# lucidrains/imagen-pytorch

Hardware: AMD Instinct MI355X
Metric: images/sec (64->256 cascade, 1000 steps, bs=8) (higher is better)
Workload: dtype f16; 1 GPU; C3: README unet1 (dim 32, 64^2) + unet2 (dim 32, 256^2, lowres_cond) cascade, 1000 DDPM steps/stage, CFG 3.0, dynamic thresholding, batch 8 per GPU; global_batch=8, parallelism=batch-sharded x1, one RCCL all-gather of final images, batch_schedule=5 whole cascades side by side (one stream each), images_in_flight=40, denoiser_evals_per_image=4000

## Files before the change

imagen-pytorch_amd/csrc/attention.hip:

```cpp
#include <cstdlib>
#include <type_traits>
#include <utility>
#include "common.h"

namespace {

constexpr int KT = 32;
constexpr int KSTR = 144;
constexpr int VSTR = 72;

template <int D>
__global__ __launch_bounds__(256) void attention_kernel(const ImagenAttentionParams p) {
  constexpr int KS = D / 16;
  constexpr int DB = D / 32;
  constexpr int KSTRD = 2 * D + 16;
  constexpr int KBYTES = KT * KSTRD;
  constexpr int VBYTES = D * VSTR;
  __shared__ __attribute__((aligned(16))) char smem[2 * (KBYTES + VBYTES)];
  const int tid = threadIdx.x, lane = tid & 63, wave = tid >> 6;
  const int half = lane >> 5, l31 = lane & 31;
  const int b = blockIdx.z, hd = blockIdx.y;
  const int row = blockIdx.x * 128 + wave * 32 + l31;
  const int row_c = row < p.rows ? row : p.rows - 1;

  const f16* q = reinterpret_cast<const f16*>(p.q) + (size_t)b * p.q_bs + (size_t)hd * p.q_hs + (size_t)row_c * p.q_rs;
  f16x8 qf[KS];
#pragma unroll
  for (int s = 0; s < KS; ++s) qf[s] = *reinterpret_cast<const f16x8*>(q + 16 * s + 8 * half);
  if (p.q_scale) {
    float ssq = 0.f;
#pragma unroll
    for (int s = 0; s < KS; ++s)
#pragma unroll
      for (int j = 0; j < 8; ++j) ssq += (float)qf[s][j] * (float)qf[s][j];
    ssq += __shfl_xor(ssq, 32);
    const float inv = p.q_mult / fmaxf(sqrtf(ssq), 1e-12f);
#pragma unroll
    for (int s = 0; s < KS; ++s) {
      const float4 g0 = *reinterpret_cast<const float4*>(p.q_scale + 16 * s + 8 * half);
      const float4 g1 = *reinterpret_cast<const float4*>(p.q_scale + 16 * s + 8 * half + 4);
      const float g[8] = {g0.x, g0.y, g0.z, g0.w, g1.x, g1.y, g1.z, g1.w};
#pragma unroll
      for (int j = 0; j < 8; ++j) qf[s][j] = (f16)((float)qf[s][j] * inv * g[j]);
    }
  }

  const f16* kg = reinterpret_cast<const f16*>(p.k) + (size_t)b * p.k_bs + (size_t)hd * p.k_hs;
  const f16* vg = reinterpret_cast<const f16*>(p.vt) + (size_t)b * p.vt_bs + (size_t)hd * p.vt_hs;
  const bool stager = tid < 4 * D;
  const int sk_key = tid / (D / 8), sk_dg = tid % (D / 8);
  const int sv_d = (tid >> 2) & (D - 1), sv_kg = tid & 3;

  uint4 k_stage = make_uint4(0, 0, 0, 0), v_stage = make_uint4(0, 0, 0, 0);
  auto tile_load = [&](int kt0) {
    if (stager) {
      k_stage = *reinterpret_cast<const uint4*>(kg + (size_t)(kt0 + sk_key) * p.k_rs + sk_dg * 8);
      v_stage = *reinterpret_cast<const uint4*>(vg + (size_t)sv_d * p.vt_ds + kt0 + sv_kg * 8);
    }
  };
  auto tile_store = [&](char* buf) {
    if (stager) {
      *reinterpret_cast<uint4*>(buf + sk_key * KSTRD + sk_dg * 16) = k_stage;
      uint2* vd = reinterpret_cast<uint2*>(buf + KBYTES + sv_d * VSTR + sv_kg * 16);
      vd[0] = make_uint2(v_stage.x, v_stage.y);
      vd[1] = make_uint2(v_stage.z, v_stage.w);
    }
  };

  f32x16 oacc[DB];
#pragma unroll
  for (int db = 0; db < DB; ++db)
#pragma unroll
    for (int r = 0; r < 16; ++r) oacc[db][r] = 0.f;
  float m_run = -1.0e30f, l_run = 0.f;

  const int ntiles = (p.J + KT - 1) / KT;
  tile_load(0);
  tile_store(smem);
  __syncthreads();
  int cur = 0;
  for (int t = 0; t < ntiles; ++t) {
    const bool more = t + 1 < ntiles;
    if (more) tile_load((t + 1) * KT);
    const char* kb = smem + cur * (KBYTES + VBYTES);
    const char* vb = kb + KBYTES;

    f32x16 sacc;
#pragma unroll
    for (int r = 0; r < 16; ++r) sacc[r] = 0.f;
#pragma unroll
    for (int s = 0; s < KS; ++s) {
      const f16x8 kf = *reinterpret_cast<const f16x8*>(kb + l31 * KSTRD + (16 * s + 8 * half) * 2);
      sacc = __builtin_amdgcn_mfma_f32_32x32x16_f16(kf, qf[s], sacc, 0, 0, 0);
    }
    const int kbase = t * KT + 4 * half;
    float mx = -1.0e30f;
#pragma unroll
    for (int r = 0; r < 16; ++r) {
      const int key = kbase + (r & 3) + 8 * (r >> 2);
      if (key >= p.J) sacc[r] = -1.0e30f;
      mx = fmaxf(mx, sacc[r]);
    }
    mx = fmaxf(mx, __shfl_xor(mx, 32));
    const float m_new = fmaxf(m_run, mx);
    const float alpha = exp2f(m_run - m_new);
    m_run = m_new;
    float psum = 0.f;
    f16x8 pf[2], pl[2];
#pragma unroll
    for (int r = 0; r < 16; ++r) {
      const float e = exp2f(sacc[r] - m_new);
      psum += e;
      const f16 eh = (f16)e;
      pf[r >> 3][r & 7] = eh;
      pl[r >> 3][r & 7] = (f16)(e - (float)eh);
    }
    l_run = l_run * alpha + psum;
#pragma unroll
    for (int db = 0; db < DB; ++db)
#pragma unroll
      for (int r = 0; r < 16; ++r) oacc[db][r] *= alpha;

#pragma unroll
    for (int s = 0; s < 2; ++s) {
#pragma unroll
      for (int db = 0; db < DB; ++db) {
        const char* vrow = vb + (32 * db + l31) * VSTR + (16 * s + 4 * half) * 2;
        const uint2 lo = *reinterpret_cast<const uint2*>(vrow);
        const uint2 hi = *reinterpret_cast<const uint2*>(vrow + 16);
        uint4 packed = make_uint4(lo.x, lo.y, hi.x, hi.y);
        const f16x8 vf = *reinterpret_cast<const f16x8*>(&packed);
        oacc[db] = __builtin_amdgcn_mfma_f32_32x32x16_f16(vf, pl[s], oacc[db], 0, 0, 0);
        oacc[db] = __builtin_amdgcn_mfma_f32_32x32x16_f16(vf, pf[s], oacc[db], 0, 0, 0);
      }
    }

    if (more) tile_store(smem + (cur ^ 1) * (KBYTES + VBYTES));
    __syncthreads();
    cur ^= 1;
  }

  const float l_tot = l_run + __shfl_xor(l_run, 32);
  const float inv = 1.0f / l_tot;
  if (row < p.rows) {
    f16* o = reinterpret_cast<f16*>(p.o) + (size_t)b * p.o_bs + (size_t)hd * p.o_hs + (size_t)row * p.o_rs;
#pragma unroll
    for (int db = 0; db < DB; ++db)
#pragma unroll
      for (int qd = 0; qd < 4; ++qd) {
        f16x4 v;
#pragma unroll
        for (int e = 0; e < 4; ++e) v[e] = (f16)(oacc[db][4 * qd + e] * inv);
        *reinterpret_cast<f16x4*>(o + 32 * db + 8 * qd + 4 * half) = v;
      }
  }
}

constexpr int KT2 = 64;
constexpr int VSTR2 = 144;
constexpr int KBYTES2 = KT2 * KSTR;
constexpr int VBYTES2 = 64 * VSTR2;

template <int MINW, int SUB>
__global__ __launch_bounds__(512, MINW) void attention_kernel_w8(const ImagenAttentionParams p) {
  extern __shared__ __attribute__((aligned(16))) char smem[];
  constexpr int SLOT = KBYTES2 + VBYTES2;
  const int tid = threadIdx.x, lane = tid & 63, wave = tid >> 6;
  const int half = lane >> 5, l31 = lane & 31;
  const int b = blockIdx.z, hd = blockIdx.y;
  const int row = blockIdx.x * 256 + wave * 32 + l31;
  const int row_c = row < p.rows ? row : p.rows - 1;

  const f16* q = reinterpret_cast<const f16*>(p.q) + (size_t)b * p.q_bs + (size_t)hd * p.q_hs + (size_t)row_c * p.q_rs;
  f16x8 qf[4];
#pragma unroll
  for (int s = 0; s < 4; ++s) qf[s] = *reinterpret_cast<const f16x8*>(q + 16 * s + 8 * half);
  if (p.q_scale) {
    float ssq = 0.f;
#pragma unroll
    for (int s = 0; s < 4; ++s)
#pragma unroll
      for (int j = 0; j < 8; ++j) ssq += (float)qf[s][j] * (float)qf[s][j];
    ssq += __shfl_xor(ssq, 32);
    const float inv = p.q_mult / fmaxf(sqrtf(ssq), 1e-12f);
#pragma unroll
    for (int s = 0; s < 4; ++s) {
      const float4 g0 = *reinterpret_cast<const float4*>(p.q_scale + 16 * s + 8 * half);
      const float4 g1 = *reinterpret_cast<const float4*>(p.q_scale + 16 * s + 8 * half + 4);
      const float g[8] = {g0.x, g0.y, g0.z, g0.w, g1.x, g1.y, g1.z, g1.w};
#pragma unroll
      for (int j = 0; j < 8; ++j) qf[s][j] = (f16)((float)qf[s][j] * inv * g[j]);
    }
  }

  const f16* kg = reinterpret_cast<const f16*>(p.k) + (size_t)b * p.k_bs + (size_t)hd * p.k_hs;
  const f16* vg = reinterpret_cast<const f16*>(p.vt) + (size_t)b * p.vt_bs + (size_t)hd * p.vt_hs;
  const int sk_key = tid >> 3, sk_dg = tid & 7;
  const int sv_d = tid >> 3, sv_kg = tid & 7;
  const int Jpad = (p.J + 31) & ~31;
  const int ntiles = (p.J + KT2 - 1) / KT2;

  uint4 ks0, vs0, ks1, vs1;
  auto one_load = [&](int t, uint4& ks, uint4& vs) __attribute__((always_inline)) {
    const int kt0 = t < ntiles ? t * KT2 : 0;
    const int kk = kt0 + sk_key < Jpad ? kt0 + sk_key : kt0;
    const int kv = kt0 + sv_kg * 8 < Jpad ? kt0 + sv_kg * 8 : kt0;
    ks = *reinterpret_cast<const uint4*>(kg + (size_t)kk * p.k_rs + sk_dg * 8);
    vs = *reinterpret_cast<const uint4*>(vg + (size_t)sv_d * p.vt_ds + kv);
  };
  auto one_store = [&](char* buf, const uint4& ks, const uint4& vs) __attribute__((always_inline)) {
    *reinterpret_cast<uint4*>(buf + sk_key * KSTR + sk_dg * 16) = ks;
    char* vrow = buf + KBYTES2 + sv_d * VSTR2 + (sv_kg >> 1) * 32 + (sv_kg & 1) * 8;
    *reinterpret_cast<uint2*>(vrow) = make_uint2(vs.x, vs.y);
    *reinterpret_cast<uint2*>(vrow + 16) = make_uint2(vs.z, vs.w);
  };
  auto group_load = [&](int t0) __attribute__((always_inline)) {
    one_load(t0, ks0, vs0);
    if constexpr (SUB > 1) one_load(t0 + 1, ks1, vs1);
  };
  auto group_store = [&](char* buf) __attribute__((always_inline)) {
    one_store(buf, ks0, vs0);
    if constexpr (SUB > 1) one_store(buf + SLOT, ks1, vs1);
  };

  f32x16 oacc[2];
#pragma unroll
  for (int db = 0; db < 2; ++db)
#pragma unroll
    for (int r = 0; r < 16; ++r) oacc[db][r] = 0.f;
  float m_run = -1.0e30f, l_run = 0.f;

  group_load(0);
  group_store(smem);
  __syncthreads();
  int cur = 0;
  for (int t0 = 0; t0 < ntiles; t0 += SUB) {
    const bool more = t0 + SUB < ntiles;
    if (more) group_load(t0 + SUB);
#pragma unroll
    for (int u = 0; u < SUB; ++u) {
      const int t = t0 + u;
      if (u > 0 && t >= ntiles) continue;
      const char* kb = smem + (cur * SUB + u) * SLOT;
      const char* vb = kb + KBYTES2;

      f32x16 sacc[2];
#pragma unroll
      for (int h2 = 0; h2 < 2; ++h2) {
#pragma unroll
        for (int r = 0; r < 16; ++r) sacc[h2][r] = 0.f;
#pragma unroll
        for (int s = 0; s < 4; ++s) {
          const f16x8 kf = *reinterpret_cast<const f16x8*>(kb + (32 * h2 + l31) * KSTR + (16 * s + 8 * half) * 2);
          sacc[h2] = __builtin_amdgcn_mfma_f32_32x32x16_f16(kf, qf[s], sacc[h2], 0, 0, 0);
        }
      }
      if (t == ntiles - 1) {
#pragma unroll
        for (int h2 = 0; h2 < 2; ++h2)
#pragma unroll
          for (int r = 0; r < 16; ++r) {
            const int key = t * KT2 + 32 * h2 + 4 * half + (r & 3) + 8 * (r >> 2);
            if (key >= p.J) sacc[h2][r] = -1.0e30f;
          }
      }
      float mx = sacc[0][0];
#pragma unroll
      for (int h2 = 0; h2 < 2; ++h2)
#pragma unroll
        for (int r = 0; r < 16; ++r) mx = fmaxf(mx, sacc[h2][r]);
      mx = fmaxf(mx, __shfl_xor(mx, 32));
      const float m_new = fmaxf(m_run, mx);
      if (__any(m_new > m_run)) {
        const float alpha = __builtin_amdgcn_exp2f(m_run - m_new);
        l_run *= alpha;
#pragma unroll
        for (int db = 0; db < 2; ++db)
#pragma unroll
          for (int r = 0; r < 16; ++r) oacc[db][r] *= alpha;
        m_run = m_new;
      }
      float psum = 0.f;
      f16x8 pf[4];
#pragma unroll
      for (int h2 = 0; h2 < 2; ++h2)
#pragma unroll
        for (int r = 0; r < 16; ++r) {
          const float e = __builtin_amdgcn_exp2f(sacc[h2][r] - m_run);
          psum += e;
          pf[2 * h2 + (r >> 3)][r & 7] = (f16)e;
        }
      l_run += psum;

#pragma unroll
      for (int h2 = 0; h2 < 2; ++h2)
#pragma unroll
        for (int s = 0; s < 2; ++s) {
#pragma unroll
          for (int db = 0; db < 2; ++db) {
            const f16x8 vf = *reinterpret_cast<const f16x8*>(vb + (32 * db + l31) * VSTR2 + (32 * h2 + 16 * s + 8 * half) * 2);
            oacc[db] = __builtin_amdgcn_mfma_f32_32x32x16_f16(vf, pf[2 * h2 + s], oacc[db], 0, 0, 0);
          }
        }
    }
    if (more) group_store(smem + (cur ^ 1) * SUB * SLOT);
    __syncthreads();
    cur ^= 1;
  }

  const float l_tot = l_run + __shfl_xor(l_run, 32);
  const float inv = 1.0f / l_tot;
  if (row < p.rows) {
    f16* o = reinterpret_cast<f16*>(p.o) + (size_t)b * p.o_bs + (size_t)hd * p.o_hs + (size_t)row * p.o_rs;
#pragma unroll
    for (int db = 0; db < 2; ++db)
#pragma unroll
      for (int qd = 0; qd < 4; ++qd) {
        f16x4 v;
#pragma unroll
        for (int e = 0; e < 4; ++e) v[e] = (f16)(oacc[db][4 * qd + e] * inv);
        *reinterpret_cast<f16x4*>(o + 32 * db + 8 * qd + 4 * half) = v;
      }
  }
}

constexpr int BND_RING = 4;

template <class F, int... I>
__device__ __forceinline__ void att_static_for_impl(F&& f, std::integer_sequence<int, I...>) {
  (f(std::integral_constant<int, I>{}), ...);
}
template <int N, class F>
__device__ __forceinline__ void att_static_for(F&& f) {
  att_static_for_impl(static_cast<F&&>(f), std::make_integer_sequence<int, N>{});
}

struct AttFrag { f16x8 k[4], v[4]; };

__device__ __forceinline__ void att_frag_load(AttFrag& f, const char* krow, const char* vrow) {
#pragma unroll
  for (int s = 0; s < 4; ++s) f.k[s] = *reinterpret_cast<const f16x8*>(krow + 32 * s);
#pragma unroll
  for (int k = 0; k < 4; ++k) f.v[k] = *reinterpret_cast<const f16x8*>(vrow + (k & 1) * 32 * VSTR2 + (k >> 1) * 32);
}

template <bool QK, bool PV>
__device__ __forceinline__ void att_bnd_step(f32x16& Sn, f32x16& Sc, f16x8 (&pc)[2], const f16x8 (&pp)[2], f32x16 (&oacc)[2], float& sum0, float& sum1,
                                             const f16x8 (&qf)[4], const AttFrag& fc, AttFrag& fn, const char* krow_next, const char* vrow_next) {
  __builtin_amdgcn_sched_barrier(0);
  IMAGEN_OPAQUE(Sc);
  att_frag_load(fn, krow_next, vrow_next);
#pragma unroll
  for (int r = 0; r < 16; ++r) {
    const float e = __builtin_amdgcn_exp2f(Sc[r]);
    if (r & 1) sum1 += e; else sum0 += e;
    pc[r >> 3][r & 7] = (f16)e;
  }
  f32x16 zero;
#pragma unroll
  for (int r = 0; r < 16; ++r) zero[r] = 0.f;
#pragma unroll
  for (int k = 0; k < 4; ++k) {
    if constexpr (QK) Sn = __builtin_amdgcn_mfma_f32_32x32x16_f16(fc.k[k], qf[k], k == 0 ? zero : Sn, 0, 0, 0);
    if constexpr (PV) oacc[k & 1] = __builtin_amdgcn_mfma_f32_32x32x16_f16(fc.v[k], pp[k >> 1], oacc[k & 1], 0, 0, 0);
  }
  constexpr int NM = (QK ? 4 : 0) + (PV ? 4 : 0);
  att_static_for<NM>([&](auto kc) __attribute__((always_inline)) {
    __builtin_amdgcn_sched_group_barrier(0x008, 1, 0);
    __builtin_amdgcn_sched_group_barrier(0x100, 8 / NM, 0);
    __builtin_amdgcn_sched_group_barrier(0x400, 16 / NM, 0);
    __builtin_amdgcn_sched_group_barrier(0x002, NM == 8 ? 3 : 6, 0);
  });
  __builtin_amdgcn_sched_barrier(0);
}

template <int NW>
__global__ __launch_bounds__(64 * NW, 2) void attention_kernel_bnd(const ImagenAttentionParams p) {
  extern __shared__ __attribute__((aligned(16))) char smem[];
  constexpr int SLOT = KBYTES2 + VBYTES2;
  constexpr int NT = 64 * NW, IT = 512 / NT;
  static_assert(IT * NT == 512 && IT <= 2, "512 items per tile, one or two per thread");
  const int tid = threadIdx.x, lane = tid & 63, wave = tid >> 6;
  const int half = lane >> 5, l31 = lane & 31;
  const int b = blockIdx.z, hd = blockIdx.y;
  const int row = blockIdx.x * (32 * NW) + wave * 32 + l31;
  const int row_c = row < p.rows ? row : p.rows - 1;

  const f16* q = reinterpret_cast<const f16*>(p.q) + (size_t)b * p.q_bs + (size_t)hd * p.q_hs + (size_t)row_c * p.q_rs;
  f16x8 qf[4];
#pragma unroll
  for (int s = 0; s < 4; ++s) qf[s] = *reinterpret_cast<const f16x8*>(q + 16 * s + 8 * half);
  if (p.q_scale) {
    float ssq = 0.f;
#pragma unroll
    for (int s = 0; s < 4; ++s)
#pragma unroll
      for (int j = 0; j < 8; ++j) ssq += (float)qf[s][j] * (float)qf[s][j];
    ssq += __shfl_xor(ssq, 32);
    const float inv = p.q_mult / fmaxf(sqrtf(ssq), 1e-12f);
#pragma unroll
    for (int s = 0; s < 4; ++s) {
      const float4 g0 = *reinterpret_cast<const float4*>(p.q_scale + 16 * s + 8 * half);
      const float4 g1 = *reinterpret_cast<const float4*>(p.q_scale + 16 * s + 8 * half + 4);
      const float g[8] = {g0.x, g0.y, g0.z, g0.w, g1.x, g1.y, g1.z, g1.w};
#pragma unroll
      for (int j = 0; j < 8; ++j) qf[s][j] = (f16)((float)qf[s][j] * inv * g[j]);
    }
  }

  const f16* kg = reinterpret_cast<const f16*>(p.k) + (size_t)b * p.k_bs + (size_t)hd * p.k_hs;
  const f16* vg = reinterpret_cast<const f16*>(p.vt) + (size_t)b * p.vt_bs + (size_t)hd * p.vt_hs;
  const int Jpad = (p.J + 31) & ~31;
  const int ntiles = (p.J + KT2 - 1) / KT2;
  struct Stage { uint4 k0, v0, k1, v1; };
  Stage st0, st1;
  auto load_item = [&](int kt0, int i, uint4& kd, uint4& vd) __attribute__((always_inline)) {
    const int key = i >> 3, g8 = i & 7;
    const int kk = kt0 + key < Jpad ? kt0 + key : kt0;
    const int kv = kt0 + g8 * 8 < Jpad ? kt0 + g8 * 8 : kt0;
    kd = *reinterpret_cast<const uint4*>(kg + (size_t)kk * p.k_rs + g8 * 8);
    vd = *reinterpret_cast<const uint4*>(vg + (size_t)key * p.vt_ds + kv);
  };
  auto store_item = [&](char* buf, int i, const uint4& kd, const uint4& vd) __attribute__((always_inline)) {
    const int key = i >> 3, g8 = i & 7;
    *reinterpret_cast<uint4*>(buf + key * KSTR + g8 * 16) = kd;
    char* vrow = buf + KBYTES2 + key * VSTR2 + (g8 >> 1) * 32 + (g8 & 1) * 8;
    *reinterpret_cast<uint2*>(vrow) = make_uint2(vd.x, vd.y);
    *reinterpret_cast<uint2*>(vrow + 16) = make_uint2(vd.z, vd.w);
  };
  auto one_load = [&](int t, Stage& st) __attribute__((always_inline)) {
    const int kt0 = (t < ntiles ? t : ntiles - 1) * KT2;
    load_item(kt0, tid, st.k0, st.v0);
    if constexpr (IT > 1) load_item(kt0, tid + NT, st.k1, st.v1);
  };
  auto one_store = [&](char* buf, const Stage& st) __attribute__((always_inline)) {
    store_item(buf, tid, st.k0, st.v0);
    if constexpr (IT > 1) store_item(buf, tid + NT, st.k1, st.v1);
  };
  auto slot = [&](int t) __attribute__((always_inline)) { return smem + (t & (BND_RING - 1)) * SLOT; };
  const int koff = l31 * KSTR + 16 * half, voff = KBYTES2 + l31 * VSTR2 + 16 * half;
  auto krow = [&](int t, int hh) __attribute__((always_inline)) { return slot(t) + koff + hh * 32 * KSTR; };
  auto vrow = [&](int t, int hh) __attribute__((always_inline)) { return slot(t) + voff + hh * 64; };
  auto mask_last = [&](f32x16& S, int t, int hh) __attribute__((always_inline)) {
#pragma unroll
    for (int r = 0; r < 16; ++r) {
      const int key = t * KT2 + 32 * hh + 4 * half + (r & 3) + 8 * (r >> 2);
      if (key >= p.J) S[r] = -1.0e30f;
    }
  };

  f32x16 oacc[2], S0, S1;
#pragma unroll
  for (int db = 0; db < 2; ++db)
#pragma unroll
    for (int r = 0; r < 16; ++r) oacc[db][r] = 0.f;
  f16x8 pA[2], pB[2];
#pragma unroll
  for (int s = 0; s < 2; ++s)
#pragma unroll
    for (int j = 0; j < 8; ++j) pA[s][j] = pB[s][j] = (f16)0.f;
  float sum0 = 0.f, sum1 = 0.f;
  AttFrag fA, fB;

  {
    Stage st2;
    one_load(0, st0);
    one_load(1, st1);
    one_load(2, st2);
    one_store(slot(0), st0);
    one_store(slot(1), st1);
    one_store(slot(2), st2);
    one_load(3, st1);
  }
  __syncthreads();
  {
#pragma unroll
    for (int r = 0; r < 16; ++r) S0[r] = 0.f;
    att_frag_load(fA, krow(0, 0), vrow(0, 0));
#pragma unroll
    for (int s = 0; s < 4; ++s) S0 = __builtin_amdgcn_mfma_f32_32x32x16_f16(fA.k[s], qf[s], S0, 0, 0, 0);
    if (ntiles == 1) mask_last(S0, 0, 0);
    att_frag_load(fA, krow(0, 1), vrow(0, 0));
    att_bnd_step<true, false>(S1, S0, pA, pB, oacc, sum0, sum1, qf, fA, fB, krow(ntiles > 1 ? 1 : 0, 0), vrow(0, 0));
    if (ntiles == 1) mask_last(S1, 0, 1);
  }
  auto iter = [&](int t, auto last_c, auto par_c) __attribute__((always_inline)) {
    constexpr bool LAST = decltype(last_c)::value;
    constexpr int PAR = decltype(par_c)::value;
    if constexpr (!LAST) {
      if constexpr (PAR == 0) one_load(t + 4, st0); else one_load(t + 4, st1);
    }
    att_bnd_step<true, true>(S0, S1, pB, pA, oacc, sum0, sum1, qf, fB, fA, krow(t + 1, 1), vrow(t, 1));
    if constexpr (LAST) mask_last(S0, t + 1, 0);
    att_bnd_step<true, true>(S1, S0, pA, pB, oacc, sum0, sum1, qf, fA, fB, krow(LAST ? t + 1 : t + 2, 0), vrow(t + 1, 0));
    if constexpr (LAST) mask_last(S1, t + 1, 1);
    if constexpr (!LAST) {
      if constexpr (PAR == 0) one_store(slot(t + 3), st1); else one_store(slot(t + 3), st0);
    }
    __syncthreads();
  };
  for (int t = 0; t + 2 < ntiles; t += 2) {
    iter(t, std::false_type{}, std::integral_constant<int, 0>{});
    if (t + 3 < ntiles) iter(t + 1, std::false_type{}, std::integral_constant<int, 1>{});
  }
  if (ntiles > 1) iter(ntiles - 2, std::true_type{}, std::integral_constant<int, 0>{});
  {
    att_bnd_step<false, true>(S0, S1, pB, pA, oacc, sum0, sum1, qf, fB, fA, krow(ntiles - 1, 1), vrow(ntiles - 1, 1));
#pragma unroll
    for (int k = 0; k < 4; ++k) oacc[k & 1] = __builtin_amdgcn_mfma_f32_32x32x16_f16(fA.v[k], pB[k >> 1], oacc[k & 1], 0, 0, 0);
  }

  float l_run = sum0 + sum1;
  const float l_tot = l_run + __shfl_xor(l_run, 32);
  const float inv = 1.0f / l_tot;
  if (row < p.rows) {
    f16* o = reinterpret_cast<f16*>(p.o) + (size_t)b * p.o_bs + (size_t)hd * p.o_hs + (size_t)row * p.o_rs;
#pragma unroll
    for (int db = 0; db < 2; ++db)
#pragma unroll
      for (int qd = 0; qd < 4; ++qd) {
        f16x4 v;
#pragma unroll
        for (int e = 0; e < 4; ++e) v[e] = (f16)(oacc[db][4 * qd + e] * inv);
        *reinterpret_cast<f16x4*>(o + 32 * db + 8 * qd + 4 * half) = v;
      }
  }
}

}

int launch_attention(const ImagenAttentionParams* p, hipStream_t s) {
  IMAGEN_CHECK(p->rows > 0 && p->J > 0 && p->B > 0 && p->heads > 0, "attention: empty problem");
  IMAGEN_CHECK(p->q_rs % 8 == 0 && p->k_rs % 8 == 0 && p->vt_ds % 8 == 0 && p->o_rs % 4 == 0,
               "attention: strides must keep 16B alignment");
  IMAGEN_CHECK(p->head_dim == 0 || p->head_dim == 64 || p->head_dim == 32, "attention: head_dim %d (64 or 32)", p->head_dim);
  IMAGEN_CHECK(p->softmax_mode == 0 || p->softmax_mode == 1, "attention: softmax_mode %d", p->softmax_mode);
  if (p->head_dim != 32 && p->rows >= 256) {
    dim3 grid((p->rows + 255) / 256, p->heads, p->B);
    auto launch = [&](auto kern, int lds, int threads = 512) {
      static bool attr_done[16] = {};
      int dev = 0;
      (void)hipGetDevice(&dev);
      if (dev < 0 || dev >= 16 || !attr_done[dev]) {
        (void)hipFuncSetAttribute(reinterpret_cast<const void*>(kern), hipFuncAttributeMaxDynamicSharedMemorySize, lds);
        if (dev >= 0 && dev < 16) attr_done[dev] = true;
      }
      hipLaunchKernelGGL(kern, grid, dim3(threads), lds, s, *p);
    };
    constexpr int slot = KBYTES2 + VBYTES2;
    if (p->softmax_mode == 1) {
      IMAGEN_CHECK(p->logit_bound > 0.0f && p->logit_bound <= 14.0f, "attention: softmax_mode 1 needs a logit bound in (0, 14] log2 units (got %g): use softmax_mode 0", (double)p->logit_bound);
      grid = dim3((p->rows + 127) / 128, p->heads, p->B);
      launch(attention_kernel_bnd<4>, BND_RING * slot, 256);
      return imagen_hip_status("attention");
    }
    if (p->J <= 2 * KT2) launch(attention_kernel_w8<4, 1>, 2 * slot);
    else launch(attention_kernel_w8<4, 2>, 4 * slot);
    return imagen_hip_status("attention");
  }
  dim3 grid((p->rows + 127) / 128, p->heads, p->B);
  if (p->head_dim == 32) hipLaunchKernelGGL(attention_kernel<32>, grid, dim3(256), 0, s, *p);
  else hipLaunchKernelGGL(attention_kernel<64>, grid, dim3(256), 0, s, *p);
  return imagen_hip_status("attention");
}
```

imagen-pytorch_amd/csrc/sampler.hip:

```cpp
#include "common.h"

namespace {

constexpr int kCoefStride = 8;

__global__ __launch_bounds__(256) void cfg_x0_kernel(const ImagenCfgX0Params p) {
  const size_t n = (size_t)p.B * p.n_per_sample;
  const size_t i = (size_t)blockIdx.x * 256 + threadIdx.x;
  if (i >= n) return;
  const float* cf = p.coef + (size_t)(*p.step_ptr) * kCoefStride;
  const float alpha = cf[0], sigma = cf[1];
  float eps;
  if (p.cfg) {
    const float cond = p.pred[i], nul = p.pred[n + i];
    eps = nul + (cond - nul) * p.cond_scale;
  } else {
    eps = p.pred[i];
  }
  float x0;
  if (p.objective == 0) x0 = (p.x[i] - sigma * eps) / fmaxf(alpha, 1e-8f);
  else if (p.objective == 1) x0 = eps;
  else x0 = alpha * p.x[i] - sigma * eps;
  p.x0[i] = x0;
  p.absx0[i] = fabsf(x0);
}

constexpr int kScratch = IMAGEN_QUANTILE_SCRATCH_WORDS;

struct Narrow { uint32_t prefix; uint32_t k; };

__device__ Narrow narrow_block(const uint32_t* hist, int passes_done, uint32_t k, uint32_t* s_scan) {
  Narrow nr{0u, k};
  const int tid = threadIdx.x, lane = tid & 63, wave = tid >> 6;
  for (int ps = 0; ps < passes_done; ++ps) {
    const uint32_t c = hist[ps * 256 + tid];
    uint32_t v = c;
#pragma unroll
    for (int off = 1; off < 64; off <<= 1) {
      const uint32_t t = __shfl_up(v, off);
      if (lane >= off) v += t;
    }
    if (lane == 63) s_scan[wave] = v;
    if (tid == 0) { s_scan[4] = 255u; s_scan[5] = 0xFFFFFFFFu; }
    __syncthreads();
    uint32_t base = 0;
    for (int w = 0; w < wave; ++w) base += s_scan[w];
    const uint32_t incl = v + base, excl = incl - c;
    if (excl <= nr.k && nr.k < incl) { s_scan[4] = (uint32_t)tid; s_scan[5] = excl; }
    __syncthreads();
    const uint32_t bin = s_scan[4];
    uint32_t cum = s_scan[5];
    if (cum == 0xFFFFFFFFu) cum = s_scan[0] + s_scan[1] + s_scan[2] + s_scan[3] - hist[ps * 256 + 255];
    __syncthreads();
    nr.prefix |= bin << (24 - 8 * ps);
    nr.k -= cum;
  }
  return nr;
}

__device__ __forceinline__ uint32_t rank_below(int n, float q) {
  const float rank = q * (float)(n - 1);
  return (uint32_t)floorf(rank);
}

__global__ __launch_bounds__(256) void quantile_hist_kernel(const ImagenQuantileParams p, int pass, int blocks_per_sample) {
  __shared__ uint32_t s_hist[256];
  __shared__ uint32_t s_scan[8];
  const int b = blockIdx.x / blocks_per_sample, blk = blockIdx.x % blocks_per_sample;
  uint32_t* scratch = p.scratch + (size_t)b * kScratch;
  s_hist[threadIdx.x] = 0;
  const Narrow nr = narrow_block(scratch, pass, rank_below(p.n, p.q), s_scan);
  __syncthreads();
  const uint32_t prefix = nr.prefix;
  const uint32_t himask = pass == 0 ? 0u : (0xFFFFFFFFu << (32 - 8 * pass));
  const int shift = 24 - 8 * pass;
  const uint32_t* keys = reinterpret_cast<const uint32_t*>(p.absx0) + (size_t)b * p.n;
  for (int i = blk * 256 + threadIdx.x; i < p.n; i += blocks_per_sample * 256) {
    const uint32_t key = keys[i];
    if ((key & himask) == (prefix & himask)) atomicAdd(&s_hist[(key >> shift) & 255u], 1u);
  }
  __syncthreads();
  const uint32_t c = s_hist[threadIdx.x];
  if (c) atomicAdd(&scratch[pass * 256 + threadIdx.x], c);
}

__global__ __launch_bounds__(256) void quantile_tail_kernel(const ImagenQuantileParams p, int blocks_per_sample) {
  __shared__ uint32_t s_scan[8];
  __shared__ uint32_t s_cnt, s_min;
  const int b = blockIdx.x / blocks_per_sample, blk = blockIdx.x % blocks_per_sample;
  uint32_t* scratch = p.scratch + (size_t)b * kScratch;
  if (threadIdx.x == 0) {
    s_cnt = 0;
    s_min = 0xFFFFFFFFu;
  }
  const Narrow nr = narrow_block(scratch, 4, rank_below(p.n, p.q), s_scan);
  __syncthreads();
  const uint32_t vlo = nr.prefix;
  const uint32_t* keys = reinterpret_cast<const uint32_t*>(p.absx0) + (size_t)b * p.n;
  uint32_t cnt = 0, mn = 0xFFFFFFFFu;
  for (int i = blk * 256 + threadIdx.x; i < p.n; i += blocks_per_sample * 256) {
    const uint32_t key = keys[i];
    if (key <= vlo) ++cnt;
    else mn = min(mn, key);
  }
  atomicAdd(&s_cnt, cnt);
  atomicMin(&s_min, mn);
  __syncthreads();
  if (threadIdx.x == 0) {
    atomicAdd(&scratch[1024], s_cnt);
    atomicMin(&scratch[1025], s_min);
  }
}

__global__ __launch_bounds__(256) void quantile_final_kernel(const ImagenQuantileParams p) {
  __shared__ uint32_t s_scan[8];
  const int b = blockIdx.x;
  uint32_t* scratch = p.scratch + (size_t)b * kScratch;
  const float rank = p.q * (float)(p.n - 1);
  const uint32_t k = (uint32_t)floorf(rank);
  const float w = rank - floorf(rank);
  const Narrow nr = narrow_block(scratch, 4, k, s_scan);
  const uint32_t cnt_le = scratch[1024], min_gt = scratch[1025];
  __syncthreads();
  for (int i = threadIdx.x; i < 1026; i += 256) scratch[i] = (i == 1025) ? 0xFFFFFFFFu : 0u;
  if (threadIdx.x == 0) {
    const uint32_t hi_key = (cnt_le >= k + 2u || min_gt == 0xFFFFFFFFu) ? nr.prefix : min_gt;
    const float lo = __uint_as_float(nr.prefix), hi = __uint_as_float(hi_key);
    const float d = hi - lo;
    p.out[b] = (w < 0.5f) ? fmaf(w, d, lo) : fmaf(w - 1.0f, d, hi);
  }
}

__device__ __forceinline__ void philox_round(uint32_t& c0, uint32_t& c1, uint32_t& c2, uint32_t& c3, uint32_t k0, uint32_t k1) {
  const uint32_t M0 = 0xD2511F53u, M1 = 0xCD9E8D57u;
  const uint32_t hi0 = __umulhi(M0, c0), lo0 = M0 * c0;
  const uint32_t hi1 = __umulhi(M1, c2), lo1 = M1 * c2;
  const uint32_t n0 = hi1 ^ c1 ^ k0, n1 = lo1, n2 = hi0 ^ c3 ^ k1, n3 = lo0;
  c0 = n0; c1 = n1; c2 = n2; c3 = n3;
}

__device__ __forceinline__ void philox_normal4(uint32_t ctr0, uint32_t ctr1, uint32_t ctr2, uint32_t ctr3, uint32_t seed_lo, uint32_t seed_hi,
                                               float out[4]) {
  uint32_t c0 = ctr0, c1 = ctr1, c2 = ctr2, c3 = ctr3, k0 = seed_lo, k1 = seed_hi;
#pragma unroll
  for (int r = 0; r < 10; ++r) {
    philox_round(c0, c1, c2, c3, k0, k1);
    k0 += 0x9E3779B9u;
    k1 += 0xBB67AE85u;
  }
  const float inv = 2.3283064365386963e-10f;
  const float u0 = ((float)c0 + 0.5f) * inv, u1 = ((float)c1 + 0.5f) * inv;
  const float u2 = ((float)c2 + 0.5f) * inv, u3 = ((float)c3 + 0.5f) * inv;
  const float r0 = sqrtf(-2.0f * __logf(fmaxf(u0, 1e-12f))), r1 = sqrtf(-2.0f * __logf(fmaxf(u2, 1e-12f)));
  float s0, c0f, s1, c1f;
  __sincosf(6.283185307179586f * u1, &s0, &c0f);
  __sincosf(6.283185307179586f * u3, &s1, &c1f);
  out[0] = r0 * c0f; out[1] = r0 * s0; out[2] = r1 * c1f; out[3] = r1 * s1;
}

__global__ __launch_bounds__(256) void ddpm_update_kernel(const ImagenDdpmUpdateParams p) {
  const size_t n = (size_t)p.B * p.n_per_sample;
  const size_t i4 = ((size_t)blockIdx.x * 256 + threadIdx.x) * 4;
  if (i4 >= n) return;
  const int step = *p.step_ptr;
  const float* cf = p.coef + (size_t)step * kCoefStride;
  const float alpha = cf[0], alpha_next = cf[2], sigma_next = cf[3], c = cf[4], nonzero = cf[5];
  const float var = sigma_next * sigma_next * c;
  const float stdev = sqrtf(fmaxf(var, 1e-20f));
  float z[4];
  if (p.noise) {
#pragma unroll
    for (int e = 0; e < 4; ++e) z[e] = (i4 + e < n) ? p.noise[i4 + e] : 0.f;
  } else {
    const int bs = (int)(i4 / p.n_per_sample);
    const uint32_t within = (uint32_t)((i4 - (size_t)bs * p.n_per_sample) >> 2);
    uint32_t k0, k1, sidx;
    if (p.row_keys) {
      k0 = p.row_keys[4 * bs], k1 = p.row_keys[4 * bs + 1], sidx = p.row_keys[4 * bs + 2];
    } else {
      k0 = p.seed_ptr ? p.seed_ptr[0] : p.seed_lo, k1 = p.seed_ptr ? p.seed_ptr[1] : p.seed_hi, sidx = (uint32_t)(p.sample_offset + bs);
    }
    philox_normal4(within, (uint32_t)step, p.stream_id, sidx, k0, k1, z);
  }
  const bool last = step + 1 >= p.total_steps;
#pragma unroll
  for (int e = 0; e < 4; ++e) {
    const size_t i = i4 + e;
    if (i >= n) break;
    const int b = (int)(i / p.n_per_sample);
    float x0 = p.x0[i];
    if (p.dynamic_threshold) {
      const float s = fmaxf(p.quant[b], 1.0f);
      x0 = fminf(fmaxf(x0, -s), s) / s;
    } else {
      x0 = fminf(fmaxf(x0, -1.0f), 1.0f);
    }
    if (p.x0_thr) p.x0_thr[i] = x0;
    const float xt = p.x[i];
    const float mean = alpha_next * (xt * (1.0f - c) / alpha + c * x0);
    const float xn = mean + nonzero * stdev * z[e];
    p.x[i] = xn;
    if (last && p.final_out) p.final_out[i] = (fminf(fmaxf(xn, -1.0f), 1.0f) + 1.0f) * 0.5f;
  }
}

__global__ void step_advance_kernel(int32_t* step_ptr) { *step_ptr += 1; }

__global__ __launch_bounds__(256) void randn_kernel(const ImagenRandnParams p) {
  const size_t n = (size_t)p.B * p.n_per_sample;
  const size_t i4 = ((size_t)blockIdx.x * 256 + threadIdx.x) * 4;
  if (i4 >= n) return;
  const int bs = (int)(i4 / p.n_per_sample);
  const uint32_t within = (uint32_t)((i4 - (size_t)bs * p.n_per_sample) >> 2);
  float z[4];
  philox_normal4(within, p.tag, p.stream_id, (uint32_t)(p.sample_offset + bs), p.seed_lo, p.seed_hi, z);
#pragma unroll
  for (int e = 0; e < 4; ++e) p.out[i4 + e] = z[e];
}

__global__ __launch_bounds__(256) void lowres_prep_kernel(const ImagenLowresPrepParams p) {
  const size_t n = (size_t)p.B * p.C * p.Hout * p.Wout;
  const size_t i = (size_t)blockIdx.x * 256 + threadIdx.x;
  if (i >= n) return;
  const int xo = (int)(i % p.Wout);
  const int yo = (int)((i / p.Wout) % p.Hout);
  const size_t bc = i / ((size_t)p.Wout * p.Hout);
  const int ys = min((int)floorf((float)yo * ((float)p.Hin / (float)p.Hout)), p.Hin - 1);
  const int xs = min((int)floorf((float)xo * ((float)p.Win / (float)p.Wout)), p.Win - 1);
  const float v = p.img[(bc * p.Hin + ys) * p.Win + xs] * 2.0f - 1.0f;
  p.out[i] = p.alpha * v + p.sigma * p.noise[i];
}

__global__ __launch_bounds__(256) void lincomb_kernel(const ImagenLincombParams p) {
  const size_t n = (size_t)p.B * p.n_per_sample;
  const size_t i4 = ((size_t)blockIdx.x * 256 + threadIdx.x) * 4;
  if (i4 >= n) return;
  const int step = *p.step_ptr;
  const float* w = p.coef + (size_t)step * 8;
  const float w0 = w[0], w1 = w[1], w2 = w[2], w3 = w[3], w4 = w[4], w5 = w[5];
  const int b = (int)(i4 / p.n_per_sample);
  float z[4] = {0.f, 0.f, 0.f, 0.f};
  if (w4 != 0.0f) {
    const uint32_t within = (uint32_t)((i4 - (size_t)b * p.n_per_sample) >> 2);
    const uint32_t k0 = p.seed_ptr ? p.seed_ptr[0] : p.seed_lo, k1 = p.seed_ptr ? p.seed_ptr[1] : p.seed_hi;
    philox_normal4(within, (uint32_t)step, p.stream_id, (uint32_t)(p.sample_offset + b), k0, k1, z);
  }
  const float s1 = (p.thr_mode == 1 && p.q1) ? fmaxf(p.q1[b], 1.0f) : 1.0f;
  const float s3 = (p.thr_mode == 1 && p.q3) ? fmaxf(p.q3[b], 1.0f) : 1.0f;
#pragma unroll
  for (int e = 0; e < 4; ++e) {
    const size_t i = i4 + e;
    float v = w0 * p.t0[i] + w4 * z[e];
    if (p.t1) {
      float t = p.t1[i];
      if (p.thr_mode) t = fminf(fmaxf(t, -s1), s1) / s1;
      v += w1 * t;
    }
    if (p.t2) v += w2 * p.t2[i];
    if (p.t3) {
      float t = p.t3[i];
      if (p.thr_mode) t = fminf(fmaxf(t, -s3), s3) / s3;
      v += w3 * t;
    }
    if (p.mask && p.mask[i] == 0.0f) v = p.mask_else[i];
    p.out[i] = v;
    if (p.out2) p.out2[i] = w5 * v;
    if (p.final && p.final_out) p.final_out[i] = (fminf(fmaxf(v, -1.0f), 1.0f) + 1.0f) * 0.5f;
  }
}

}

int launch_lincomb(const ImagenLincombParams* p, hipStream_t s) {
  IMAGEN_CHECK(p->t0 && p->out && p->coef && p->step_ptr, "lincomb: t0 / out / coef / step_ptr required");
  IMAGEN_CHECK(p->n_per_sample % 4 == 0 && p->B > 0, "lincomb: n_per_sample %% 4");
  IMAGEN_CHECK(!p->mask || p->mask_else, "lincomb: mask needs mask_else");
  const size_t n = (size_t)p->B * p->n_per_sample;
  hipLaunchKernelGGL(lincomb_kernel, dim3((unsigned)((n / 4 + 255) / 256)), dim3(256), 0, s, *p);
  if (p->advance) hipLaunchKernelGGL(step_advance_kernel, dim3(1), dim3(1), 0, s, p->step_ptr);
  return imagen_hip_status("lincomb");
}

int launch_cfg_x0(const ImagenCfgX0Params* p, hipStream_t s) {
  IMAGEN_CHECK(p->step_ptr && p->coef, "cfg_x0: coef table / step counter required");
  const size_t n = (size_t)p->B * p->n_per_sample;
  hipLaunchKernelGGL(cfg_x0_kernel, dim3((unsigned)((n + 255) / 256)), dim3(256), 0, s, *p);
  return imagen_hip_status("cfg_x0");
}

int launch_quantile(const ImagenQuantileParams* p, hipStream_t s) {
  IMAGEN_CHECK(p->n >= 2 && p->B > 0, "quantile: need n >= 2");
  int bps = (p->n + 8191) / 8192;
  if (bps < 1) bps = 1;
  if (bps > 64) bps = 64;
  for (int pass = 0; pass < 4; ++pass)
    hipLaunchKernelGGL(quantile_hist_kernel, dim3(p->B * bps), dim3(256), 0, s, *p, pass, bps);
  hipLaunchKernelGGL(quantile_tail_kernel, dim3(p->B * bps), dim3(256), 0, s, *p, bps);
  hipLaunchKernelGGL(quantile_final_kernel, dim3(p->B), dim3(256), 0, s, *p);
  return imagen_hip_status("quantile");
}

int launch_randn(const ImagenRandnParams* p, hipStream_t s) {
  IMAGEN_CHECK(p->n_per_sample % 4 == 0, "randn: n_per_sample must be a multiple of 4");
  const size_t n4 = ((size_t)p->B * p->n_per_sample) / 4;
  hipLaunchKernelGGL(randn_kernel, dim3((unsigned)((n4 + 255) / 256)), dim3(256), 0, s, *p);
  return imagen_hip_status("randn");
}

int launch_lowres_prep(const ImagenLowresPrepParams* p, hipStream_t s) {
  const size_t n = (size_t)p->B * p->C * p->Hout * p->Wout;
  hipLaunchKernelGGL(lowres_prep_kernel, dim3((unsigned)((n + 255) / 256)), dim3(256), 0, s, *p);
  return imagen_hip_status("lowres_prep");
}

int launch_ddpm_update(const ImagenDdpmUpdateParams* p, hipStream_t s) {
  IMAGEN_CHECK(p->step_ptr && p->coef, "ddpm_update: coef table / step counter required");
  IMAGEN_CHECK(p->n_per_sample % 4 == 0, "ddpm_update: n_per_sample must be a multiple of 4");
  IMAGEN_CHECK(!p->dynamic_threshold || p->quant, "ddpm_update: dynamic thresholding needs the quantile");
  const size_t n4 = ((size_t)p->B * p->n_per_sample + 3) / 4;
  hipLaunchKernelGGL(ddpm_update_kernel, dim3((unsigned)((n4 + 255) / 256)), dim3(256), 0, s, *p);
  if (!p->no_advance) hipLaunchKernelGGL(step_advance_kernel, dim3(1), dim3(1), 0, s, p->step_ptr);
  return imagen_hip_status("ddpm_update");
}
```

Measured before the change: 1.383 images/s.

## Add single-launch LDS radix-select quantile for small images; use permlane32 swap

For per-sample sizes that fit in shared memory (up to 13312 keys), dynamic thresholding now uses one workgroup per sample. That workgroup loads the keys into LDS and runs a three-pass radix select with wave-aggregated LDS histogram atomics, then takes the next-larger key. This replaces four histogram passes, a tail kernel and a final kernel, each a separate launch through global scratch. It should apply to the 64x64 stage but not the 256x256 one. The attention epilogue also swaps the cross-half l_run reduction to permlane32_swap and recomputes the output row and half from an opaque thread id, apparently to ease register pressure.

```diff
diff --git a/imagen-pytorch_amd/csrc/attention.hip b/imagen-pytorch_amd/csrc/attention.hip
--- a/imagen-pytorch_amd/csrc/attention.hip
+++ b/imagen-pytorch_amd/csrc/attention.hip
@@ -308,10 +308,15 @@
     cur ^= 1;
   }
 
-  const float l_tot = l_run + __shfl_xor(l_run, 32);
+  int tid_e = threadIdx.x;
+  IMAGEN_OPAQUE(tid_e);
+  const int half_e = (tid_e >> 5) & 1;
+  const int row_e = blockIdx.x * 256 + (tid_e >> 6) * 32 + (tid_e & 31);
+  const auto l_pair = __builtin_amdgcn_permlane32_swap(__float_as_uint(l_run), __float_as_uint(l_run), false, false);
+  const float l_tot = __uint_as_float(l_pair[0]) + __uint_as_float(l_pair[1]);
   const float inv = 1.0f / l_tot;
-  if (row < p.rows) {
-    f16* o = reinterpret_cast<f16*>(p.o) + (size_t)b * p.o_bs + (size_t)hd * p.o_hs + (size_t)row * p.o_rs;
+  if (row_e < p.rows) {
+    f16* o = reinterpret_cast<f16*>(p.o) + (size_t)b * p.o_bs + (size_t)hd * p.o_hs + (size_t)row_e * p.o_rs;
 #pragma unroll
     for (int db = 0; db < 2; ++db)
 #pragma unroll
@@ -319,7 +324,7 @@
         f16x4 v;
 #pragma unroll
         for (int e = 0; e < 4; ++e) v[e] = (f16)(oacc[db][4 * qd + e] * inv);
-        *reinterpret_cast<f16x4*>(o + 32 * db + 8 * qd + 4 * half) = v;
+        *reinterpret_cast<f16x4*>(o + 32 * db + 8 * qd + 4 * half_e) = v;
       }
   }
 }
diff --git a/imagen-pytorch_amd/csrc/sampler.hip b/imagen-pytorch_amd/csrc/sampler.hip
--- a/imagen-pytorch_amd/csrc/sampler.hip
+++ b/imagen-pytorch_amd/csrc/sampler.hip
@@ -131,6 +131,114 @@
   }
 }
 
+constexpr int kLdsThreads = 1024;
+constexpr int kLdsKeys = 13312;
+constexpr int kLdsBins = 2048;
+
+__device__ __forceinline__ void lds_hist_add(uint32_t* hist, uint32_t bin, bool valid) {
+  const unsigned long long m = __ballot(valid);
+  if (m == 0ull) return;
+  const int leader = __ffsll(m) - 1;
+  const uint32_t first = (uint32_t)__shfl((int)bin, leader);
+  if (__ballot(valid && bin == first) == m) {
+    if ((int)(threadIdx.x & 63) == leader) atomicAdd(&hist[first], (uint32_t)__popcll(m));
+  } else if (valid) {
+    atomicAdd(&hist[bin], 1u);
+  }
+}
+
+struct Pick { uint32_t bin, below, count; };
+
+__device__ Pick lds_pick_bin(uint32_t* hist, int bins, uint32_t k, uint32_t* s_wave, uint32_t* s_pick) {
+  const int tid = threadIdx.x, lane = tid & 63, wave = tid >> 6;
+  const int per = bins / kLdsThreads;
+  const uint32_t c0 = hist[tid * per], c1 = per == 2 ? hist[tid * per + 1] : 0u;
+  uint32_t v = c0 + c1;
+#pragma unroll
+  for (int off = 1; off < 64; off <<= 1) {
+    const uint32_t t = __shfl_up(v, off);
+    if (lane >= off) v += t;
+  }
+  if (lane == 63) s_wave[wave] = v;
+  __syncthreads();
+  uint32_t base = 0;
+  for (int w = 0; w < wave; ++w) base += s_wave[w];
+  const uint32_t incl = v + base, excl = incl - (c0 + c1);
+  if (excl <= k && k < incl) {
+    const bool second = k >= excl + c0;
+    s_pick[0] = (uint32_t)(tid * per) + (second ? 1u : 0u);
+    s_pick[1] = second ? excl + c0 : excl;
+    s_pick[2] = second ? c1 : c0;
+  }
+  hist[tid * per] = 0u;
+  if (per == 2) hist[tid * per + 1] = 0u;
+  __syncthreads();
+  return Pick{s_pick[0], s_pick[1], s_pick[2]};
+}
+
+__global__ __launch_bounds__(kLdsThreads) void quantile_lds_kernel(const ImagenQuantileParams p) {
+  __shared__ __attribute__((aligned(16))) uint32_t s_keys[kLdsKeys];
+  __shared__ uint32_t s_hist[kLdsBins];
+  __shared__ uint32_t s_wave[kLdsThreads / 64];
+  __shared__ uint32_t s_pick[3];
+  __shared__ uint32_t s_min;
+  const int b = blockIdx.x, tid = threadIdx.x, n = p.n;
+  const uint32_t* keys = reinterpret_cast<const uint32_t*>(p.absx0) + (size_t)b * n;
+  if ((reinterpret_cast<uintptr_t>(keys) & 15u) == 0) {
+    const uint4* keys4 = reinterpret_cast<const uint4*>(keys);
+    uint4* s_keys4 = reinterpret_cast<uint4*>(s_keys);
+    const int n4 = n >> 2;
+    for (int i = tid; i < n4; i += kLdsThreads) s_keys4[i] = keys4[i];
+    for (int i = (n4 << 2) + tid; i < n; i += kLdsThreads) s_keys[i] = keys[i];
+  } else {
+    for (int i = tid; i < n; i += kLdsThreads) s_keys[i] = keys[i];
+  }
+  for (int i = tid; i < kLdsBins; i += kLdsThreads) s_hist[i] = 0u;
+  if (tid == 0) s_min = 0xFFFFFFFFu;
+  __syncthreads();
+
+  const float rank = p.q * (float)(n - 1);
+  const uint32_t k = (uint32_t)floorf(rank);
+  const float w = rank - floorf(rank);
+  const int n_up = (n + kLdsThreads - 1) / kLdsThreads * kLdsThreads;
+
+  uint32_t prefix = 0u, himask = 0u, krem = k, count = 0u;
+#pragma unroll
+  for (int pass = 0; pass < 3; ++pass) {
+    const int bits = pass == 2 ? 10 : 11, shift = pass == 0 ? 21 : (pass == 1 ? 10 : 0);
+    for (int i = tid; i < n_up; i += kLdsThreads) {
+      const bool in = i < n;
+      const uint32_t key = in ? s_keys[i] : 0u;
+      lds_hist_add(s_hist, (key >> shift) & ((1u << bits) - 1u), in && (key & himask) == prefix);
+    }
+    __syncthreads();
+    const Pick pk = lds_pick_bin(s_hist, 1 << bits, krem, s_wave, s_pick);
+    prefix |= pk.bin << shift;
+    himask |= ((1u << bits) - 1u) << shift;
+    krem -= pk.below;
+    count = pk.count;
+  }
+  const uint32_t vlo = prefix;
+  const uint32_t cnt_le = (k - krem) + count;
+
+  uint32_t mn = 0xFFFFFFFFu;
+  for (int i = tid; i < n; i += kLdsThreads) {
+    const uint32_t key = s_keys[i];
+    if (key > vlo) mn = min(mn, key);
+  }
+#pragma unroll
+  for (int off = 32; off > 0; off >>= 1) mn = min(mn, (uint32_t)__shfl_xor((int)mn, off));
+  if ((tid & 63) == 0 && mn != 0xFFFFFFFFu) atomicMin(&s_min, mn);
+  __syncthreads();
+  if (tid == 0) {
+    const uint32_t min_gt = s_min;
+    const uint32_t hi_key = (cnt_le >= k + 2u || min_gt == 0xFFFFFFFFu) ? vlo : min_gt;
+    const float lo = __uint_as_float(vlo), hi = __uint_as_float(hi_key);
+    const float d = hi - lo;
+    p.out[b] = (w < 0.5f) ? fmaf(w, d, lo) : fmaf(w - 1.0f, d, hi);
+  }
+}
+
 __device__ __forceinline__ void philox_round(uint32_t& c0, uint32_t& c1, uint32_t& c2, uint32_t& c3, uint32_t k0, uint32_t k1) {
   const uint32_t M0 = 0xD2511F53u, M1 = 0xCD9E8D57u;
   const uint32_t hi0 = __umulhi(M0, c0), lo0 = M0 * c0;
@@ -290,6 +398,10 @@
 
 int launch_quantile(const ImagenQuantileParams* p, hipStream_t s) {
   IMAGEN_CHECK(p->n >= 2 && p->B > 0, "quantile: need n >= 2");
+  if (p->n <= kLdsKeys) {
+    hipLaunchKernelGGL(quantile_lds_kernel, dim3(p->B), dim3(kLdsThreads), 0, s, *p);
+    return imagen_hip_status("quantile");
+  }
   int bps = (p->n + 8191) / 8192;
   if (bps < 1) bps = 1;
   if (bps > 64) bps = 64;
```

Result: no change. 1.380 images/s (-0.2%).
